# Tongji-MIC-Lab/TDVC

Hardware: AMD Instinct MI355X
Metric: 1080p P-frames/sec (encode + reconstruct, lambda=2048 config) (higher is better)
Workload: dtype f16; 1 GPU; 1x 1920x1080 (padded 1088x1920) 7-frame synthetic GOP (seed 1234), batch 1, P-frames coded in GOP order; gop=7, batch=1, parallelism=gop-sharded x1, weights=closed-form filler (no checkpoint ships)

## Files before the change

### include/tdvc_hip.h

```cpp
#ifndef TDVC_HIP_H
#define TDVC_HIP_H

#include <stdint.h>

#ifdef __cplusplus
extern "C" {
#endif

#define TDVC_OK 0
#define TDVC_EINVAL (-1)
#define TDVC_ENOSUP (-2)

typedef struct {
  void* p;
  int32_t N, H, W, C;
  int64_t sn;
  int32_t sp;
  int32_t dtype;
} tdvc_fmap;

enum { TDVC_F16 = 0, TDVC_F32 = 1 };
enum { TDVC_ACT_NONE = 0, TDVC_ACT_RELU = 1, TDVC_ACT_LRELU = 2, TDVC_ACT_CLAMP01 = 3, TDVC_ACT_SIGMOID = 4 };
enum { TDVC_GDN_NONE = 0, TDVC_GDN_FWD = 1, TDVC_GDN_INV = 2 };
enum { TDVC_OUT_NHWC = 0,
       TDVC_OUT_SHUFFLE2 = 1,
       TDVC_OUT_NCHW_F32 = 2 };

#define TDVC_MAX_TAPS 49

typedef struct {
  tdvc_fmap x;
  tdvc_fmap y;
  const void* w;
  const float* bias;
  int32_t cout;
  int32_t ntaps;
  int8_t tap_dy[TDVC_MAX_TAPS], tap_dx[TDVC_MAX_TAPS];
  int32_t kh, kw, stride, pad;
  int32_t ck;
  int32_t square_input;
  int32_t gdn;
  tdvc_fmap aux;
  int32_t act; float slope;
  int32_t round_before_act;
  tdvc_fmap res;
  tdvc_fmap res2;
  int32_t out_mode;
  int32_t s2d;
  int32_t bcast_T;
  float bcast_slope;
  float* chan_sum;
  tdvc_fmap flow;
} tdvc_conv_desc;

int tdvc_abi_version(void);
const char* tdvc_last_error(void);
int tdvc_prepare_device(void);
const char* tdvc_last_conv_kernel(void);

int tdvc_set_predicate(const int* flag);
int tdvc_last_launch_predicated(void);
#define TDVC_MAX_PREDICATE_IMAGES 4
int tdvc_set_predicate_images(const int* flags, int n);
int tdvc_frame_changed(const tdvc_fmap* cur, tdvc_fmap* cache, int* flag, void* stream);
int tdvc_frames_changed(const tdvc_fmap* cur, tdvc_fmap* cache, int* flags, unsigned force_mask, void* stream);


int tdvc_conv_plan(int cin, int kh, int kw, int stride);
int64_t tdvc_conv_packed_bytes(int cout, int cin, int ntaps, int ck);
int tdvc_pack_conv_weights(const float* w_oihw, int cout, int cin_real, int cin, int kh, int kw,
                           int ntaps, const int8_t* tap_dy, const int8_t* tap_dx, int ck, uint16_t* dst);
int tdvc_conv2d(const tdvc_conv_desc* d, void* stream);
int tdvc_conv_chan_sum_rows(const tdvc_conv_desc* d);
int tdvc_conv_flow_supported(const tdvc_conv_desc* d);
const char* tdvc_conv_select(const tdvc_conv_desc* d);
int tdvc_conv2d_f32(const tdvc_conv_desc* d, void* stream);

typedef struct {
  tdvc_fmap x, y;
  const void* w;
  const float* bias;
  int32_t act1; float slope1;
  int32_t act2; float slope2;
  int32_t add_input;
  tdvc_fmap res2;
} tdvc_conv_pair_desc;
int64_t tdvc_conv_pair_packed_bytes(void);
int tdvc_pack_conv_pair_weights(const float* w1_oihw, const float* w2_oihw, uint16_t* dst);
int tdvc_conv_pair_supported(const tdvc_conv_pair_desc* d);
int tdvc_conv_pair(const tdvc_conv_pair_desc* d, void* stream);

typedef struct {
  tdvc_fmap x, om, y;
  const void* w;
  const float* bias;
  int32_t groups;
  int32_t act; float slope; int32_t round_before_act;
  void* x_planar;
} tdvc_dcn_desc;
int tdvc_dcn_fused(const tdvc_dcn_desc* d, void* stream);

int tdvc_dcn_v2_forward_f32(const float* input, const float* weight, const float* bias,
                            const float* offset, const float* mask, float* output,
                            int B, int C, int H, int W, int Cout,
                            int kh, int kw, int sh, int sw, int ph, int pw, int dh, int dw,
                            int deformable_group, void* stream);
int tdvc_dcn_v2_backward_f32(const float* input, const float* weight, const float* bias,
                             const float* offset, const float* mask, const float* grad_output,
                             float* grad_input, float* grad_offset, float* grad_mask,
                             float* grad_weight, float* grad_bias, float* columns,
                             int B, int C, int H, int W, int Cout,
                             int kh, int kw, int sh, int sw, int ph, int pw, int dh, int dw,
                             int deformable_group, void* stream);

int tdvc_nchw_to_fmap(const float* src, int C, const tdvc_fmap* y, void* stream);
int tdvc_fmap_to_nchw(const tdvc_fmap* x, int C, float* dst, void* stream);
int tdvc_scale_act_res(const tdvc_fmap* a, const float* gate, int act, float slope,
                       const tdvc_fmap* r, float r_sign, const tdvc_fmap* y, const tdvc_fmap* y2, void* stream);
int tdvc_scale_act_res3(const tdvc_fmap* a, const float* gate, int act, float slope, const tdvc_fmap* r, float r_sign,
                        const tdvc_fmap* y, const tdvc_fmap* b, float b_sign, const tdvc_fmap* y3, void* stream);
int tdvc_add_flow(const tdvc_fmap* off, const tdvc_fmap* flow, void* stream);
int tdvc_bcast_add_act(const tdvc_fmap* x, const tdvc_fmap* b, int T, float slope, void* stream);

int tdvc_channel_sum(const tdvc_fmap* x, float* partial, int nblocks, void* stream);
int tdvc_se_gate(const float* partial, int nblocks, float inv_count, int N, int C, int Cmid,
                 const float* w1, const float* b1, const float* w2, const float* b2,
                 float* gate, void* stream);

int tdvc_upsample2x(const tdvc_fmap* x, const tdvc_fmap* y, void* stream);
int tdvc_avgpool2(const tdvc_fmap* x, const tdvc_fmap* y, void* stream);
int tdvc_avgpool2_pyramid(const tdvc_fmap* xa, const tdvc_fmap* xb, const tdvc_fmap* ya, const tdvc_fmap* yb, void* stream);
int tdvc_spynet_level_input(const tdvc_fmap* ref, const tdvc_fmap* supp, const tdvc_fmap* flow_lo,
                            const tdvc_fmap* flow_up, const tdvc_fmap* cat8, void* stream);
int tdvc_resize_bilinear(const tdvc_fmap* x, const tdvc_fmap* y, const float* chscale, void* stream);

int64_t tdvc_avgpool_k_work_floats(int N, int hp, int wp, int C, int scale);
int tdvc_avgpool_k(const tdvc_fmap* x, int scale, float* pooled, int hp, int wp, float* work, int64_t work_floats, void* stream);
int tdvc_patch_match(const float* pin, const float* pref, int N, int hp, int wp, int C,
                     int32_t* idx, void* stream);
int tdvc_match_gather(const tdvc_fmap* fin, const tdvc_fmap* fref, const int32_t* idx, int scale,
                      int hp, int wp, const tdvc_fmap* cat, void* stream);
// ... 176 lines not shown
```

### tdvc_amd/_lib.py

```python
from __future__ import annotations

import ctypes as C
import os

_HERE = os.path.dirname(os.path.abspath(__file__))
LIB_PATH = os.path.join(_HERE, "libtdvc_hip.so")

MAX_TAPS = 49
F16, F32 = 0, 1
ACT_NONE, ACT_RELU, ACT_LRELU, ACT_CLAMP01, ACT_SIGMOID = 0, 1, 2, 3, 4
GDN_NONE, GDN_FWD, GDN_INV = 0, 1, 2
OUT_NHWC, OUT_SHUFFLE2, OUT_NCHW_F32 = 0, 1, 2


class FMapDesc(C.Structure):
    _fields_ = [("p", C.c_void_p), ("N", C.c_int32), ("H", C.c_int32), ("W", C.c_int32), ("C", C.c_int32),
                ("sn", C.c_int64), ("sp", C.c_int32), ("dtype", C.c_int32)]


class ConvDesc(C.Structure):
    _fields_ = [("x", FMapDesc), ("y", FMapDesc), ("w", C.c_void_p), ("bias", C.c_void_p),
                ("cout", C.c_int32), ("ntaps", C.c_int32),
                ("tap_dy", C.c_int8 * MAX_TAPS), ("tap_dx", C.c_int8 * MAX_TAPS),
                ("kh", C.c_int32), ("kw", C.c_int32), ("stride", C.c_int32), ("pad", C.c_int32),
                ("ck", C.c_int32), ("square_input", C.c_int32), ("gdn", C.c_int32),
                ("aux", FMapDesc), ("act", C.c_int32), ("slope", C.c_float),
                ("round_before_act", C.c_int32), ("res", FMapDesc), ("res2", FMapDesc), ("out_mode", C.c_int32), ("s2d", C.c_int32),
                ("bcast_T", C.c_int32), ("bcast_slope", C.c_float), ("chan_sum", C.c_void_p), ("flow", FMapDesc)]


class DcnDesc(C.Structure):
    _fields_ = [("x", FMapDesc), ("om", FMapDesc), ("y", FMapDesc), ("w", C.c_void_p), ("bias", C.c_void_p),
                ("groups", C.c_int32), ("act", C.c_int32), ("slope", C.c_float), ("round_before_act", C.c_int32), ("x_planar", C.c_void_p)]


class ConvPairDesc(C.Structure):
    _fields_ = [("x", FMapDesc), ("y", FMapDesc), ("w", C.c_void_p), ("bias", C.c_void_p), ("act1", C.c_int32), ("slope1", C.c_float),
                ("act2", C.c_int32), ("slope2", C.c_float), ("add_input", C.c_int32), ("res2", FMapDesc)]


class WgradReduceJob(C.Structure):
    _fields_ = [("work", C.c_void_p), ("bwork", C.c_void_p), ("row_off", C.c_void_p), ("chan_off", C.c_void_p), ("tap_off", C.c_void_p),
                ("bias_index", C.c_void_p), ("dw", C.c_void_p), ("db", C.c_void_p), ("scale", C.c_float),
                ("nworkers", C.c_int32), ("cow", C.c_int32), ("ciw", C.c_int32), ("ntaps", C.c_int32), ("cout", C.c_int32), ("cin", C.c_int32),
                ("wblocks", C.c_int32), ("nblocks", C.c_int32)]


_P = C.c_void_p
_FM = C.POINTER(FMapDesc)
_i, _f, _i64 = C.c_int, C.c_float, C.c_int64

SIGNATURES = {
    "tdvc_abi_version": (_i, []),
    "tdvc_conv_chan_sum_rows": (_i, [C.POINTER(ConvDesc)]),
    "tdvc_conv_select": (C.c_char_p, [C.POINTER(ConvDesc)]),
    "tdvc_conv_flow_supported": (_i, [C.POINTER(ConvDesc)]),
    "tdvc_scale_act_res3": (_i, [_FM, _P, _i, _f, _FM, _f, _FM, _FM, _f, _FM, _P]),
    "tdvc_avgpool2_pyramid": (_i, [_FM, _FM, _FM, _FM, _P]),
    "tdvc_last_error": (C.c_char_p, []),
    "tdvc_last_conv_kernel": (C.c_char_p, []),
    "tdvc_prepare_device": (_i, []),
    "tdvc_set_predicate": (_i, [_P]),
    "tdvc_set_predicate_images": (_i, [_P, _i]),
    "tdvc_last_launch_predicated": (_i, []),
    "tdvc_frame_changed": (_i, [_FM, _FM, _P, _P]),
    "tdvc_frames_changed": (_i, [_FM, _FM, _P, C.c_uint, _P]),
    "tdvc_conv_plan": (_i, [_i, _i, _i, _i]),
    "tdvc_conv_packed_bytes": (_i64, [_i, _i, _i, _i]),
    "tdvc_pack_conv_weights": (_i, [_P, _i, _i, _i, _i, _i, _i, _P, _P, _i, _P]),
    "tdvc_conv2d": (_i, [C.POINTER(ConvDesc), _P]),
    "tdvc_conv2d_f32": (_i, [C.POINTER(ConvDesc), _P]),
    "tdvc_pack_conv_weights_indexed": (_i, [_P] * 7 + [_i] * 4 + [_P, _P]),
    "tdvc_pack_conv_weights_indexed_f32": (_i, [_P] * 7 + [_i] * 4 + [_P, _P]),
    "tdvc_pack_job_blocks": (_i64, [_i, _i, _i, _i]),
    "tdvc_pack_conv_weights_batch": (_i, [_P, _P, _i, _i, _P]),
    "tdvc_act_backward": (_i, [_FM, _FM, _FM, _i, _f, _FM, _P]),
    "tdvc_pixel_unshuffle": (_i, [_FM, _FM, _P]),
    "tdvc_bias_grad_work_floats": (_i64, [_i, _i]),
    "tdvc_bias_grad": (_i, [_FM, _i, _P, _f, _P, _P, _i64, _P]),
    "tdvc_copy_cast": (_i, [_FM, _FM, _P]),
    "tdvc_clamp01_backward": (_i, [_FM, _FM, _P]),
    "tdvc_gate_backward_work_floats": (_i64, [_i, _i]),
    "tdvc_gate_backward": (_i, [_FM, _FM, _P, _FM, _P, _P, _i64, _P]),
    "tdvc_se_gate_backward": (_i, [_P, _i, _f, _i, _i, _i] + [_P] * 6 + [_f] + [_P] * 6),
    "tdvc_bcast_channel_add": (_i, [_FM, _P, _f, _P]),
    "tdvc_add_flow_backward": (_i, [_FM, _FM, _P]),
    "tdvc_bcast_add_act_backward": (_i, [_FM, _FM, _FM, _f, _P]),
    "tdvc_upsample2x_backward": (_i, [_FM, _FM, _P]),
    "tdvc_resize_bilinear_backward": (_i, [_FM, _FM, _P, _P]),
    "tdvc_spynet_level_input_backward": (_i, [_FM, _FM, _FM, _FM, _FM, _P]),
    "tdvc_sigmoid_f32": (_i, [_P, _P, _i64, _P]),
    "tdvc_sigmoid_backward_f32": (_i, [_P, _P, _i64, _P]),
    "tdvc_axpy_f32": (_i, [_P, _P, _f, _i64, _P]),
    "tdvc_match_gather_backward": (_i, [_FM, _FM, _P, _i, _i, _i, _FM, _FM, _FM, _P]),
    "tdvc_eb_backward": (_i, [_FM, _P, _FM, _f, _FM, _P, _P]),
    "tdvc_eb_pack": (_i, [_P, _P, _P, _i, _P]),
    "tdvc_eb_param_chain": (_i, [_P, _P, _P, _f, _i, _P]),
    "tdvc_eb_aux": (_i, [_P, _P, _f, _P, _P, _i, _P]),
    "tdvc_gc_backward": (_i, [_FM, _FM, _FM, _f, _FM, _FM, _P]),
    "tdvc_dcn_columns": (_i, [_FM, _FM, _i, _FM, _P]),
    "tdvc_ar_lanes_state_bytes": (_i64, [_i]),
    "tdvc_ar_gather_batch": (_i, [_FM, _FM, _P, _i, _FM, _FM, _P]),
    "tdvc_ar_quantize_batch": (_i, [_FM, _FM, _P, _i, _P, _i, _P, _FM, _P, _P, _i64, _P]),
    "tdvc_ar_indexes_batch": (_i, [_FM, _P, _i, _i, _P, _i, _i, _i, _i, _P, _i64, _P]),
    "tdvc_ar_wavefront_batch": (_i, [_P, _P, _i, _P, _i, _P, _P, _FM, _FM, _FM, _FM, _FM, _P, _i, _FM, _P, _P, _i, _i, _i, _P, _i, _P, _P, _P]),
    "tdvc_ar_decode_serial_batch": (_i, [_P, _P, _i, _P, _i, _P, _P, _FM, _FM, _FM, _FM, _P, _i, _FM, _P, _i, _i, _i, _P, _i, _P, _P, _P]),
    "tdvc_ar_lanes_batch_layout": (_i64, [_P, _i, _i, _P]),
    "tdvc_ar_lanes_init_batch": (_i, [_P, _i64, _P, _i, _i, _P, _P]),
    "tdvc_ar_decode_lanes_step_batch": (_i, [_FM, _P, _i, _P, _i, _P, _i64, _P, _i, _P, C.c_int32, _P, _P, _P, C.c_int32, _P, _FM, _P, _P, _i64, _P]),
    "tdvc_ar_wavefront_lanes_batch": (_i, [_P, _P, _i, _P, _i64, _P, _P, C.c_int32, _P, _P, _P, C.c_int32, _FM, _FM, _FM, _FM, _P, _i, _FM, _P, _P, _i, _i, _i,
                                           _P, _i, _P, _P, _P, _P]),
    "tdvc_ar_encode_lanes_scratch_words": (_i64, [_i64, _i, _i]),
    "tdvc_ar_encode_lanes_out_bytes": (_i64, [_i64, _i, _i]),
    "tdvc_ar_encode_lanes_batch": (_i, [_P, _P, _i, _i, _i, _i, _P, _i, _i, _P, C.c_int32, _P, _P, _P, C.c_int32, _P, _i64, _i64, _P, _i64, _i64, _P, _P]),
    "tdvc_rans_encode_lanes_dev_ref": (_i, [_P, _P, _i, _i, _i, _i, _P, _i, _i, _P, C.c_int32, _P, _P, C.c_int32, _P, _i64, _i64, _P, _i64, _i64, _P]),
    "tdvc_ar_last_loop_launches": (_i64, []),
    "tdvc_ssim_level_work_floats": (_i64, [_i] * 5),
    "tdvc_ssim_level": (_i, [_P, _P, _i, _i, _i, _i, _P, _i, _f, _f, _P, _P, _P, _i64, _P]),
    "tdvc_avgpool2_pad_f32": (_i, [_P, _i64, _i, _i, _P, _P]),
    "tdvc_ssim_level_backward": (_i, [_P, _P, _i, _i, _i, _i, _P, _i, _f, _f, _P, _P, _f, _P, _P, _P]),
    "tdvc_msssim_level_grads": (_i, [_P, _P, _P, _i, _i, _P, _P, _P, _P, _P]),
    "tdvc_dcn_col2im_work_floats": (_i64, [_i, _i, _i, _i]),
    "tdvc_dcn_col2im": (_i, [_FM, _FM, _FM, _i, _P, _FM, _P, _i64, _P]),
    "tdvc_dcn_col2im_det": (_i, [_FM, _FM, _FM, _i, _P, _FM, _P, _i64, _P, _P, _P, _i, _P]),
    "tdvc_dcn_far_apply": (_i, [_P, _P, _P, _i, _P, _P]),
    "tdvc_conv_wgrad_work_floats": (_i64, [_i] * 6),
    "tdvc_conv_wgrad": (_i, [_FM, _FM] + [_i] * 6 + [_P] * 5 + [_i, _f, _P, _P, _i64, _P]),
    "tdvc_conv_wgrad_bias": (_i, [_FM, _FM] + [_i] * 6 + [_P] * 5 + [_i, _f, _P, _P, _P, _P, _i64, _P]),
    "tdvc_conv_wgrad_partials": (_i, [_FM, _FM] + [_i] * 6 + [_P] * 5 + [_i, _f, _P, _P, _P, _P, _i64, C.POINTER(WgradReduceJob), _P]),
    "tdvc_wgrad_reduce_batch": (_i, [_P, _P, _i, _i, _P]),
    "tdvc_gdn_backward": (_i, [_FM, _FM, _FM, _i, _FM, _FM, _P]),
    "tdvc_mul2_accumulate": (_i, [_FM, _FM, _FM, _P]),
    "tdvc_dcn_fused": (_i, [C.POINTER(DcnDesc), _P]),
    "tdvc_conv_pair_packed_bytes": (_i64, []),
    "tdvc_pack_conv_pair_weights": (_i, [_P, _P, _P]),
    "tdvc_conv_pair_supported": (_i, [C.POINTER(ConvPairDesc)]),
    "tdvc_conv_pair": (_i, [C.POINTER(ConvPairDesc), _P]),
    "tdvc_dcn_v2_forward_f32": (_i, [_P] * 6 + [_i] * 14 + [_P]),
    "tdvc_dcn_v2_backward_f32": (_i, [_P] * 12 + [_i] * 14 + [_P]),
    "tdvc_nchw_to_fmap": (_i, [_P, _i, _FM, _P]),
    "tdvc_fmap_to_nchw": (_i, [_FM, _i, _P, _P]),
    "tdvc_scale_act_res": (_i, [_FM, _P, _i, _f, _FM, _f, _FM, _FM, _P]),
    "tdvc_add_flow": (_i, [_FM, _FM, _P]),
# ... 57 lines not shown
```

### tdvc_amd/csrc/conv_common.h

```cpp
#pragma once
#include "common.h"

namespace convk {

struct ConvParams {
  const half_t* x; long x_sn; int x_sp; int H, W, Cin;
  const half_t* w; const float* bias;
  FMap y; int Ho, Wo; int cout;
  FMap aux; FMap res; FMap res2;
  int ntaps, kh, kw, pad;
  int in_stride;
  int nchunks, steps;
  int square, gdn, act; float slope; int round16, out_mode;
  int tiles_x;
  int simple;
  int s2d, Corig;
  int reverse;
  int bcast_T; float bcast_slope;
  float* csum;
  int8_t tap_dy[TDVC_MAX_TAPS], tap_dx[TDVC_MAX_TAPS];
  const int* pred;
  FMap flow;
};

enum ConvSwitch { SW_NONE = -1, SW_V2, SW_V3, SW_V5, SW_V7, SW_V9, SW_V10, SW_V11, SW_ROW, SW_C8, SW_N16, SW_GDN128, SW_HEAD3, SW_COUNT };
int conv_on(int id);
long conv_v9_work_limit();

constexpr long LARGE_MAP_PIXELS = 8192;

inline bool taps_dense(const tdvc_conv_desc* d, int kh, int kw, int pad) {
  if (d->ntaps != kh * kw || d->kh != kh || d->kw != kw || d->pad != pad) return false;
  for (int t = 0; t < d->ntaps; ++t)
    if (d->tap_dy[t] != t / kw || d->tap_dx[t] != t % kw) return false;
  return true;
}

inline bool all_waves_store(const tdvc_conv_desc* d, int wave_ch) {
  const int ych = d->out_mode == TDVC_OUT_SHUFFLE2 ? d->cout >> 2 : (d->cout + wave_ch - 1) / wave_ch * wave_ch;
  return d->y.C > ych - wave_ch;
}

inline int persistent_grid_x(int slots, int cout_blocks, int N, int ntiles) {
  const int gx = slots / (cout_blocks * N);
  return gx < 1 ? 1 : (gx > ntiles ? ntiles : gx);
}

template <auto Kern, typename... Args>
int launch_big_lds(const char* what, int lds_limit, dim3 grid, dim3 block, int lds, hipStream_t st, Args... args) {
  static TdvcPerDeviceFlag raised;
  bool& done = raised.flag();
  if (!done) {
    const hipError_t err = hipFuncSetAttribute(reinterpret_cast<const void*>(Kern), hipFuncAttributeMaxDynamicSharedMemorySize, lds_limit);
    if (err != hipSuccess) { tdvc_set_error("%s: hipFuncSetAttribute failed: %s", what, hipGetErrorString(err)); return (int)err; }
    done = true;
  }
  hipLaunchKernelGGL(Kern, grid, block, lds, st, args...);
  return tdvc_launch_status(what);
}


template <bool F32MAPS = false>
__device__ __forceinline__ void epilogue4(const ConvParams& p, int n, int oy, int ox, int co, float v[4]) {
  if (p.bias) {
    const f32x4 b4 = *reinterpret_cast<const f32x4*>(p.bias + co);
#pragma unroll
    for (int i = 0; i < 4; ++i) v[i] += b4[i];
  }
  int py = oy, px = ox, pc = co, PW = p.Wo;
  if (p.out_mode == TDVC_OUT_SHUFFLE2) {
    const int cq = p.cout >> 2;
    const int sub = co / cq;
    pc = co - sub * cq;
    py = 2 * oy + (sub >> 1);
    px = 2 * ox + (sub & 1);
    PW = 2 * p.Wo;
  }
  if (p.gdn) {
    float a[4];
    if (F32MAPS && p.aux.f32) {
      const f32x4 a4 = *reinterpret_cast<const f32x4*>(reinterpret_cast<const float*>(p.aux.p) + (long)n * p.aux.sn + ((long)oy * p.Wo + ox) * p.aux.sp + co);
#pragma unroll
      for (int i = 0; i < 4; ++i) v[i] = a4[i] * (p.gdn == TDVC_GDN_FWD ? 1.0f / sqrtf(v[i]) : sqrtf(v[i]));
    } else {
      const half4 a4 = *reinterpret_cast<const half4*>(reinterpret_cast<const half_t*>(p.aux.p) + (long)n * p.aux.sn + ((long)oy * p.Wo + ox) * p.aux.sp + co);
#pragma unroll
      for (int i = 0; i < 4; ++i) a[i] = (float)a4[i];
#pragma unroll
      for (int i = 0; i < 4; ++i) v[i] = a[i] * (p.gdn == TDVC_GDN_FWD ? rsqrtf(v[i]) : sqrtf(v[i]));
    }
  }
  if (p.round16) {
#pragma unroll
    for (int i = 0; i < 4; ++i) v[i] = (float)(half_t)v[i];
  }
  if (p.act) {
#pragma unroll
    for (int i = 0; i < 4; ++i) v[i] = act_apply(v[i], p.act, p.slope);
  }
  const long opix = (long)py * PW + px;
  if (p.res.p) {
    if (p.res.f32) {
      const float* rp = reinterpret_cast<const float*>(p.res.p) + (long)n * p.res.sn + opix * p.res.sp + pc;
#pragma unroll
      for (int i = 0; i < 4; ++i)
        if (pc + i < p.res.C) v[i] += rp[i];
    } else if (pc < p.res.C) {
      const half4 r4 = *reinterpret_cast<const half4*>(reinterpret_cast<const half_t*>(p.res.p) + (long)n * p.res.sn + opix * p.res.sp + pc);
// ... 326 lines not shown
```

### tdvc_amd/csrc/conv_dispatch.hip

```cpp
#include <stdlib.h>

#include "conv_common.h"

using convk::ConvParams;
bool conv_v2_eligible(const tdvc_conv_desc* d, int Ho, int Wo); int launch_conv_v2(const ConvParams& p, int cout_blocks, int N, hipStream_t st);
bool conv_v3_eligible(const tdvc_conv_desc* d, int Ho, int Wo); int launch_conv_v3(const ConvParams& p, int cout_blocks, int N, hipStream_t st);
bool conv_v5_eligible(const tdvc_conv_desc* d, int Ho, int Wo); int launch_conv_v5(const ConvParams& p, int cout_blocks, int N, hipStream_t st); int conv_v5_chan_sum_rows(int Ho, int Wo, int cout_blocks, int N);
bool conv_v7_eligible(const tdvc_conv_desc* d, const ConvParams& p, int Ho, int Wo); int launch_conv_v7(const ConvParams& p, int cout_blocks, int N, hipStream_t st);
bool conv_v9_eligible(const tdvc_conv_desc* d, int Ho, int Wo, bool v3_ok); int launch_conv_v9(const ConvParams& p, int ck8, int cout_tiles32, int N, hipStream_t st);
bool conv_v10_eligible(const tdvc_conv_desc* d, const ConvParams& p, int Ho, int Wo); int launch_conv_v10(const ConvParams& p, int cout_blocks, int N, hipStream_t st);
bool conv_v11_eligible(const tdvc_conv_desc* d, const ConvParams& p, int Ho, int Wo); int launch_conv_v11(const ConvParams& p, int cout_blocks, int N, hipStream_t st);
int conv_row_geometry(const tdvc_conv_desc* d, const ConvParams& p, int Ho, int Wo); int launch_conv_row(int geo, const ConvParams& p, int N, hipStream_t st);
bool conv_c8_eligible(const tdvc_conv_desc* d, const ConvParams& p, int Ho, int Wo); int launch_conv_c8(const ConvParams& p, int N, hipStream_t st);
bool conv_n16_eligible(const tdvc_conv_desc* d, int Ho, int Wo); int launch_conv_n16(const ConvParams& p, int N, hipStream_t st);
bool gdn128_eligible(const tdvc_conv_desc* d, const ConvParams& p, int Ho, int Wo); int launch_gdn128(const ConvParams& p, int N, hipStream_t st);
int conv_direct_lds_bytes(const tdvc_conv_desc* d);
int conv_cout_tiles(int cout);
int launch_conv_direct(const ConvParams& p, int ck8, int stride, int N, hipStream_t st);
int conv_f32_validate(const tdvc_conv_desc* d, int& Ho, int& Wo);

namespace {
const char* const kSwitchEnv[convk::SW_COUNT] = {nullptr, "TDVC_CONV_NO_V3", "TDVC_CONV_NO_V5", "TDVC_CONV_NO_V7", "TDVC_CONV_NO_V9", "TDVC_CONV_NO_V10",
                                                 "TDVC_CONV_NO_V11", "TDVC_CONV_NO_ROW", "TDVC_CONV_NO_C8", "TDVC_CONV_NO_N16", "TDVC_CONV_NO_GDN128", "TDVC_CONV_NO_HEAD3"};
int g_enabled[convk::SW_COUNT] = {1, 1, 1, 1, 1, 1, 1, 15, 1, 1, 1, 1};
long g_v9_work_limit = 1L << 20;
}

int convk::conv_on(int id) {
  static const struct EnvOff {
    bool off[convk::SW_COUNT];
    EnvOff() {
      const bool v1 = getenv("TDVC_CONV_V1") != nullptr;
      for (int i = 0; i < convk::SW_COUNT; ++i) off[i] = v1 || (kSwitchEnv[i] && getenv(kSwitchEnv[i]) != nullptr);
    }
  } env;
  return id == convk::SW_NONE ? 1 : (env.off[id] ? 0 : g_enabled[id]);
}
long convk::conv_v9_work_limit() { return g_v9_work_limit; }

extern "C" void tdvc_debug_enable_conv_v9(int enable) { g_enabled[convk::SW_V9] = enable != 0; }
extern "C" void tdvc_debug_enable_conv_v10(int enable) { g_enabled[convk::SW_V10] = enable != 0; }
extern "C" void tdvc_debug_enable_conv_v11(int enable) { g_enabled[convk::SW_V11] = enable != 0; }
extern "C" void tdvc_debug_enable_conv_row(int mask) { g_enabled[convk::SW_ROW] = mask; }
extern "C" void tdvc_debug_enable_conv_c8(int enable) { g_enabled[convk::SW_C8] = enable != 0; }
extern "C" void tdvc_debug_enable_conv_n16(int enable) { g_enabled[convk::SW_N16] = enable != 0; }
extern "C" void tdvc_debug_enable_gdn128(int enable) { g_enabled[convk::SW_GDN128] = enable != 0; }
extern "C" void tdvc_debug_enable_conv_head3(int enable) { g_enabled[convk::SW_HEAD3] = enable != 0; }
extern "C" void tdvc_debug_set_conv_v9_work_limit(long v) { g_v9_work_limit = v; }

namespace {

struct Pick {
  const tdvc_conv_desc* d;
  int Ho, Wo;
  int geo;
  int ck8() const { return d->ck / 8; }
  int N() const { return d->x.N; }
  int cout_blocks() const { return conv_cout_tiles(d->cout) / 2; }
};

struct Entry {
  const char* name;
  int sw;
  bool (*eligible)(Pick& k, const ConvParams& p);
  int (*launch)(const Pick& k, const ConvParams& p, hipStream_t st);
  bool (*only)(const tdvc_conv_desc* d);
  const char* only_msg;
};

bool v3_on_and_eligible(const Pick& k) { return convk::conv_on(convk::SW_V3) && conv_v3_eligible(k.d, k.Ho, k.Wo); }

bool bcast_eligible(Pick& k, const ConvParams& p) {
  const tdvc_conv_desc* d = k.d;
  return d->bcast_T == 4 && d->kh == 1 && d->kw == 1 && d->stride == 1 && d->pad == 0 && d->cout == 64 && d->y.C == 64 && d->y.sp >= 4 * 64 &&
         d->y.dtype == TDVC_F16 && d->out_mode == TDVC_OUT_NHWC && d->act == TDVC_ACT_NONE && !d->gdn && !d->res2.p &&
         (!d->res.p || (d->res.dtype == TDVC_F16 && d->res.C == 64 && d->res.sp >= 4 * 64 && d->res.N == d->y.N && d->res.H == d->y.H && d->res.W == d->y.W)) &&
         !d->square_input && !d->round_before_act && d->bias && d->bcast_slope >= 0.f && d->bcast_slope <= 1.f && conv_v5_eligible(d, k.Ho, k.Wo) &&
         convk::conv_is_lean(p);
}
int bcast_launch(const Pick& k, const ConvParams& p, hipStream_t st) {
  ConvParams q = p;
  q.simple = 2;
  q.slope = 1.f;
  return launch_conv_v5(q, 1, k.N(), st);
}
bool row_eligible(Pick& k, const ConvParams& p) { return (k.geo = conv_row_geometry(k.d, p, k.Ho, k.Wo)) >= 0; }

constexpr char kNameV5[] = "conv_mfma_v5", kNameDirect[] = "conv_mfma<%d,%d,%d>";

const Entry kTable[] = {
    {"conv_mfma_v5(bcast)", convk::SW_V5, bcast_eligible, bcast_launch, [](const tdvc_conv_desc* d) { return d->bcast_T != 0; },
     "tdvc_conv2d: bcast_T needs a plain 1x1 / stride 1 conv to 64 channels of >= 8192 pixels, y (and res, the optional source of the slices) a 64-channel window of a buffer with >= 4 slices, bcast_T == 4"},
    {"conv_row(s2d)", convk::SW_ROW, [](Pick& k, const ConvParams& p) { return k.d->s2d && row_eligible(k, p); },
     [](const Pick& k, const ConvParams& p, hipStream_t st) { return launch_conv_row(k.geo, p, k.N(), st); }, nullptr, nullptr},
    {"conv_mfma_v3(s2d)", convk::SW_V3, [](Pick& k, const ConvParams&) { return k.d->s2d && conv_v3_eligible(k.d, k.Ho, k.Wo); },
     [](const Pick& k, const ConvParams& p, hipStream_t st) { return launch_conv_v3(p, k.cout_blocks(), k.N(), st); },
     [](const tdvc_conv_desc* d) { return d->s2d != 0; }, "tdvc_conv2d: s2d conv not eligible for the stage-pipelined kernel"},
    {"conv_mfma_v9", convk::SW_V9, [](Pick& k, const ConvParams&) { return conv_v9_eligible(k.d, k.Ho, k.Wo, v3_on_and_eligible(k)); },
     [](const Pick& k, const ConvParams& p, hipStream_t st) { return launch_conv_v9(p, k.ck8(), conv_cout_tiles(k.d->cout), k.N(), st); }, nullptr, nullptr},
    {"gdn128", convk::SW_GDN128, [](Pick& k, const ConvParams& p) { return gdn128_eligible(k.d, p, k.Ho, k.Wo); },
     [](const Pick& k, const ConvParams& p, hipStream_t st) { return launch_gdn128(p, k.N(), st); }, nullptr, nullptr},
    {kNameV5, convk::SW_V5, [](Pick& k, const ConvParams&) { return conv_v5_eligible(k.d, k.Ho, k.Wo); },
     [](const Pick& k, const ConvParams& p, hipStream_t st) { return launch_conv_v5(p, k.cout_blocks(), k.N(), st); }, nullptr, nullptr},
    {"conv_c8", convk::SW_C8, [](Pick& k, const ConvParams& p) { return conv_c8_eligible(k.d, p, k.Ho, k.Wo); },
     [](const Pick& k, const ConvParams& p, hipStream_t st) { return launch_conv_c8(p, k.N(), st); }, nullptr, nullptr},
    {"conv_n16", convk::SW_N16, [](Pick& k, const ConvParams&) { return conv_n16_eligible(k.d, k.Ho, k.Wo); },
     [](const Pick& k, const ConvParams& p, hipStream_t st) { return launch_conv_n16(p, k.N(), st); }, nullptr, nullptr},
    {"conv_row", convk::SW_ROW, row_eligible,
     [](const Pick& k, const ConvParams& p, hipStream_t st) { return launch_conv_row(k.geo, p, k.N(), st); }, nullptr, nullptr},
    {"conv_mfma_v10", convk::SW_V10, [](Pick& k, const ConvParams& p) { return conv_v10_eligible(k.d, p, k.Ho, k.Wo); },
     [](const Pick& k, const ConvParams& p, hipStream_t st) { return launch_conv_v10(p, k.cout_blocks(), k.N(), st); }, nullptr, nullptr},
    {"conv_mfma_v7", convk::SW_V7, [](Pick& k, const ConvParams& p) { return conv_v7_eligible(k.d, p, k.Ho, k.Wo); },
     [](const Pick& k, const ConvParams& p, hipStream_t st) { return launch_conv_v7(p, k.cout_blocks(), k.N(), st); }, nullptr, nullptr},
    {"conv_mfma_v11", convk::SW_V11, [](Pick& k, const ConvParams& p) { return conv_v11_eligible(k.d, p, k.Ho, k.Wo); },
     [](const Pick& k, const ConvParams& p, hipStream_t st) { return launch_conv_v11(p, k.cout_blocks(), k.N(), st); }, nullptr, nullptr},
    {"conv_mfma_v3", convk::SW_V3, [](Pick& k, const ConvParams&) { return conv_v3_eligible(k.d, k.Ho, k.Wo); },
     [](const Pick& k, const ConvParams& p, hipStream_t st) { return launch_conv_v3(p, k.cout_blocks(), k.N(), st); }, nullptr, nullptr},
    {"conv_mfma_v2", convk::SW_V2, [](Pick& k, const ConvParams&) { return conv_v2_eligible(k.d, k.Ho, k.Wo); },
     [](const Pick& k, const ConvParams& p, hipStream_t st) { return launch_conv_v2(p, k.cout_blocks(), k.N(), st); }, nullptr, nullptr},
    {kNameDirect, convk::SW_NONE, [](Pick& k, const ConvParams&) { return conv_direct_lds_bytes(k.d) <= 64 * 1024; },
     [](const Pick& k, const ConvParams& p, hipStream_t st) { return launch_conv_direct(p, k.ck8(), k.d->stride, k.N(), st); },
     [](const tdvc_conv_desc*) { return true; }, nullptr},
};

const Entry* select(Pick& k, const ConvParams& p) {
  for (const Entry& e : kTable) {
    if (convk::conv_on(e.sw) && e.eligible(k, p)) return &e;
    if (e.only && e.only(k.d)) {
      if (e.only_msg) tdvc_set_error("%s", e.only_msg);
      else tdvc_set_error("tdvc_conv2d: LDS plan %d bytes too large for the direct kernel (use tdvc_conv_plan)", conv_direct_lds_bytes(k.d));
// ... 162 lines not shown
```

### tdvc_amd/csrc/conv_n16.hip

```cpp
#include "conv_common.h"

using convk::ConvParams;

namespace {

constexpr int N16_TH = 8, N16_TW = 64, N16_NTHR = 512;

struct N16Extra {
  int ksteps;
  int ps;
  int a_bytes;
  int ntiles, tiles_x;
  int cin_shift;
};

template <int NCB>
__global__ __launch_bounds__(N16_NTHR, 1) void conv_n16_kernel(const ConvParams p, const N16Extra e) {
  extern __shared__ __attribute__((aligned(16))) unsigned char smem[];
  unsigned char* wl = smem;
  unsigned char* tile = wl + e.a_bytes;
  const int tid = threadIdx.x, lane = tid & 63;
  const int wave = __builtin_amdgcn_readfirstlane(tid >> 6);
  const int px = lane & 15, kg = lane >> 4;
  const int TIW = N16_TW + p.kw - 1, TIH = N16_TH + p.kh - 1;
// ... 16 lines not shown
    return base + (dy * TIW + dx) * e.ps + (kk0 & (cin - 1)) * 2;
  };

  for (int tile_i = blockIdx.x; tile_i < e.ntiles; tile_i += gridDim.x) {
    const int per_img = e.tiles_x * ((p.Ho + N16_TH - 1) / N16_TH);
    const int n = tile_i / per_img, rem = tile_i - n * per_img;
    const int ty = rem / e.tiles_x, tx = rem - ty * e.tiles_x;
    const half_t* xn = p.x + (long)n * p.x_sn;
    const int iy0 = ty * N16_TH - p.pad, ix0 = tx * N16_TW - p.pad;
    __syncthreads();
    const int total = TIH * TIW * c8n;
    for (int idx0 = tid; idx0 < total; idx0 += 8 * N16_NTHR) {
      half8 v[8];
#pragma unroll
      for (int u = 0; u < 8; ++u) {
        const int idx = idx0 + u * N16_NTHR;
        const int pix = idx >> (e.cin_shift - 3), c8 = idx & (c8n - 1);
        const int rr = pix / TIW, cc = pix - rr * TIW;
        const int iy = iy0 + rr, ix = ix0 + cc;
        const bool ok = (int)(idx < total) & (int)(iy >= 0) & (int)(iy < p.H) & (int)(ix >= 0) & (int)(ix < p.W);
        const half_t* src = xn + ((long)(ok ? iy : 0) * p.W + (ok ? ix : 0)) * p.x_sp + c8 * 8;
        typedef unsigned u32x4 __attribute__((ext_vector_type(4)));
        u32x4 bits = *reinterpret_cast<const u32x4*>(src);
        unsigned m = ok ? 0xFFFFFFFFu : 0u;
        asm volatile("" : "+v"(m));
        bits &= m;
        v[u] = __builtin_bit_cast(half8, bits);
      }
#pragma unroll
      for (int u = 0; u < 8; ++u) {
        const int idx = idx0 + u * N16_NTHR;
        if (idx < total) {
          const int pix = idx >> (e.cin_shift - 3), c8 = idx & (c8n - 1);
          *reinterpret_cast<half8*>(tile + pix * e.ps + c8 * 16) = v[u];
        }
      }
    }
    __syncthreads();

    f32x4 acc[NCB][4];
#pragma unroll
    for (int cb = 0; cb < NCB; ++cb)
#pragma unroll
      for (int c = 0; c < 4; ++c) acc[cb][c] = f32x4{0.f, 0.f, 0.f, 0.f};

    half8 a0[NCB], b0[4], a1[NCB], b1[4];
    auto load = [&](int S, half8 (&a)[NCB], half8 (&b)[4]) {
      const int off = frag_off(S);
#pragma unroll
      for (int cb = 0; cb < NCB; ++cb) a[cb] = *reinterpret_cast<const half8*>(wl + ((S * NCB + cb) * 64 + lane) * 16);
#pragma unroll
      for (int c = 0; c < 4; ++c) b[c] = *reinterpret_cast<const half8*>(tile + off + c * cstep);
    };
    auto mm = [&](half8 (&a)[NCB], half8 (&b)[4]) {
#pragma unroll
      for (int c = 0; c < 4; ++c)
#pragma unroll
        for (int cb = 0; cb < NCB; ++cb) acc[cb][c] = __builtin_amdgcn_mfma_f32_16x16x32_f16(a[cb], b[c], acc[cb][c], 0, 0, 0);
    };
    const int KS = e.ksteps;
    load(0, a0, b0);
    for (int S = 0; S < KS; S += 2) {
      load(min(S + 1, KS - 1), a1, b1);
      mm(a0, b0);
      load(min(S + 2, KS - 1), a0, b0);
      if (S + 1 < KS) mm(a1, b1);
    }

    const int oy = ty * N16_TH + wave;
#pragma unroll
    for (int c = 0; c < 4; ++c) {
      const int ox = tx * N16_TW + 16 * c + px;
      if (oy < p.Ho && ox < p.Wo) {
#pragma unroll
        for (int cb = 0; cb < NCB; ++cb) {
          float v[4] = {acc[cb][c][0], acc[cb][c][1], acc[cb][c][2], acc[cb][c][3]};
          convk::epilogue4(p, n, oy, ox, 16 * cb + 4 * kg, v);
        }
      }
    }
  }
}

inline int n16_ps(int cin) { return 2 * cin + 16; }
inline int n16_ksteps(int ntaps, int cin) { return (ntaps * cin + 31) / 32; }
inline int n16_lds(int cin, int kh, int kw, int ntaps, int ncb) {
  return n16_ksteps(ntaps, cin) * ncb * 1024 + (N16_TH + kh - 1) * (N16_TW + kw - 1) * n16_ps(cin);
}

}

bool conv_n16_eligible(const tdvc_conv_desc* d, int Ho, int Wo) {
  const int cin = d->x.C;
  const bool cin_ok = cin == 8 || cin == 16 || cin == 32 || cin == 64;
  const bool dense = convk::taps_dense(d, d->kh, d->kw, d->pad);
  return cin_ok && dense && d->ck == cin && d->stride == 1 && d->cout <= 32 && !d->s2d && !d->square_input && !d->gdn &&
         (long)Ho * Wo >= convk::LARGE_MAP_PIXELS &&
         n16_lds(cin, d->kh, d->kw, d->ntaps, d->cout <= 16 ? 1 : 2) <= 150 * 1024;
}

bool conv_head3_takes(const ConvParams& p);
int launch_conv_head3(const ConvParams& p, int N, hipStream_t st);
static thread_local int g_n16_last_form = 0;
extern "C" int tdvc_debug_conv_n16_last_form(void) { return g_n16_last_form; }

int launch_conv_n16(const ConvParams& p, int N, hipStream_t st) {
  g_n16_last_form = convk::conv_on(convk::SW_HEAD3) && conv_head3_takes(p);
  if (g_n16_last_form) return launch_conv_head3(p, N, st);
  const int ncb = p.cout <= 16 ? 1 : 2;
  N16Extra e;
  e.ksteps = n16_ksteps(p.ntaps, p.Cin);
  e.ps = n16_ps(p.Cin);
  e.a_bytes = e.ksteps * ncb * 1024;
  e.tiles_x = (p.Wo + N16_TW - 1) / N16_TW;
  e.ntiles = N * e.tiles_x * ((p.Ho + N16_TH - 1) / N16_TH);
  e.cin_shift = p.Cin == 8 ? 3 : p.Cin == 16 ? 4 : p.Cin == 32 ? 5 : 6;
  const int lds = n16_lds(p.Cin, p.kh, p.kw, p.ntaps, ncb);
  const int per_cu = lds <= 78 * 1024 ? 2 : 1;
  int grid = e.ntiles < 256 * per_cu ? e.ntiles : 256 * per_cu;
  const auto go = ncb == 1 ? convk::launch_big_lds<&conv_n16_kernel<1>, ConvParams, N16Extra> : convk::launch_big_lds<&conv_n16_kernel<2>, ConvParams, N16Extra>;
  return go("tdvc_conv2d(n16)", 160 * 1024, dim3(grid), dim3(N16_NTHR), lds, st, p, e);
}
```

Measured before the change: 52.15 frames/s.

## Add register-prefetched streaming variant of n16 conv kernel overlapping next tile loads

Adds a persistent n16 conv kernel that loads the next tile's input into registers while the MFMA loop for the current tile runs, then writes it to LDS after a barrier. Bias is preloaded into registers and added before the epilogue. The goal is to hide global-load latency between tiles in the persistent loop. The cost is more register pressure from PT prefetch vectors under launch_bounds(…,1), plus an extra barrier per tile. The kernel is enabled by default, and a debug knob to force per-CU occupancy is added.

```diff
diff --git a/include/tdvc_hip.h b/include/tdvc_hip.h
--- a/include/tdvc_hip.h
+++ b/include/tdvc_hip.h
@@ -57,6 +57,8 @@
 const char* tdvc_last_error(void);
 int tdvc_prepare_device(void);
 const char* tdvc_last_conv_kernel(void);
+void tdvc_debug_enable_conv_n16_stream(int enable);
+int tdvc_debug_conv_n16_last_stream(void);
 
 int tdvc_set_predicate(const int* flag);
 int tdvc_last_launch_predicated(void);
diff --git a/tdvc_amd/_lib.py b/tdvc_amd/_lib.py
--- a/tdvc_amd/_lib.py
+++ b/tdvc_amd/_lib.py
@@ -59,6 +59,8 @@
     "tdvc_avgpool2_pyramid": (_i, [_FM, _FM, _FM, _FM, _P]),
     "tdvc_last_error": (C.c_char_p, []),
     "tdvc_last_conv_kernel": (C.c_char_p, []),
+    "tdvc_debug_enable_conv_n16_stream": (None, [_i]),
+    "tdvc_debug_conv_n16_last_stream": (_i, []),
     "tdvc_prepare_device": (_i, []),
     "tdvc_set_predicate": (_i, [_P]),
     "tdvc_set_predicate_images": (_i, [_P, _i]),
diff --git a/tdvc_amd/csrc/conv_common.h b/tdvc_amd/csrc/conv_common.h
--- a/tdvc_amd/csrc/conv_common.h
+++ b/tdvc_amd/csrc/conv_common.h
@@ -23,7 +23,7 @@
   FMap flow;
 };
 
-enum ConvSwitch { SW_NONE = -1, SW_V2, SW_V3, SW_V5, SW_V7, SW_V9, SW_V10, SW_V11, SW_ROW, SW_C8, SW_N16, SW_GDN128, SW_HEAD3, SW_COUNT };
+enum ConvSwitch { SW_NONE = -1, SW_V2, SW_V3, SW_V5, SW_V7, SW_V9, SW_V10, SW_V11, SW_ROW, SW_C8, SW_N16, SW_GDN128, SW_HEAD3, SW_N16_STREAM, SW_COUNT };
 int conv_on(int id);
 long conv_v9_work_limit();
 
diff --git a/tdvc_amd/csrc/conv_dispatch.hip b/tdvc_amd/csrc/conv_dispatch.hip
--- a/tdvc_amd/csrc/conv_dispatch.hip
+++ b/tdvc_amd/csrc/conv_dispatch.hip
@@ -21,8 +21,9 @@
 
 namespace {
 const char* const kSwitchEnv[convk::SW_COUNT] = {nullptr, "TDVC_CONV_NO_V3", "TDVC_CONV_NO_V5", "TDVC_CONV_NO_V7", "TDVC_CONV_NO_V9", "TDVC_CONV_NO_V10",
-                                                 "TDVC_CONV_NO_V11", "TDVC_CONV_NO_ROW", "TDVC_CONV_NO_C8", "TDVC_CONV_NO_N16", "TDVC_CONV_NO_GDN128", "TDVC_CONV_NO_HEAD3"};
-int g_enabled[convk::SW_COUNT] = {1, 1, 1, 1, 1, 1, 1, 15, 1, 1, 1, 1};
+                                                 "TDVC_CONV_NO_V11", "TDVC_CONV_NO_ROW", "TDVC_CONV_NO_C8", "TDVC_CONV_NO_N16", "TDVC_CONV_NO_GDN128", "TDVC_CONV_NO_HEAD3",
+                                                 "TDVC_CONV_NO_N16_STREAM"};
+int g_enabled[convk::SW_COUNT] = {1, 1, 1, 1, 1, 1, 1, 15, 1, 1, 1, 1, 1};
 long g_v9_work_limit = 1L << 20;
 }
 
@@ -46,6 +47,7 @@
 extern "C" void tdvc_debug_enable_conv_n16(int enable) { g_enabled[convk::SW_N16] = enable != 0; }
 extern "C" void tdvc_debug_enable_gdn128(int enable) { g_enabled[convk::SW_GDN128] = enable != 0; }
 extern "C" void tdvc_debug_enable_conv_head3(int enable) { g_enabled[convk::SW_HEAD3] = enable != 0; }
+extern "C" void tdvc_debug_enable_conv_n16_stream(int enable) { g_enabled[convk::SW_N16_STREAM] = enable != 0; }
 extern "C" void tdvc_debug_set_conv_v9_work_limit(long v) { g_v9_work_limit = v; }
 
 namespace {
diff --git a/tdvc_amd/csrc/conv_n16.hip b/tdvc_amd/csrc/conv_n16.hip
--- a/tdvc_amd/csrc/conv_n16.hip
+++ b/tdvc_amd/csrc/conv_n16.hip
@@ -122,6 +122,140 @@
   }
 }
 
+template <int NCB, int PT>
+__global__ __launch_bounds__(N16_NTHR, 1) void conv_n16_stream_kernel(const ConvParams p, const N16Extra e) {
+  typedef unsigned u32x4 __attribute__((ext_vector_type(4)));
+  extern __shared__ __attribute__((aligned(16))) unsigned char smem[];
+  unsigned char* wl = smem;
+  unsigned char* tile = wl + e.a_bytes;
+  const int tid = threadIdx.x, lane = tid & 63;
+  const int wave = __builtin_amdgcn_readfirstlane(tid >> 6);
+  const int px = lane & 15, kg = lane >> 4;
+  const int TIW = N16_TW + p.kw - 1, TIH = N16_TH + p.kh - 1;
+  const int cin = p.Cin, c8n = cin >> 3;
+  const int total = TIH * TIW * c8n;
+  const int per_img = e.tiles_x * ((p.Ho + N16_TH - 1) / N16_TH);
+
+  u32x4 treg[PT];
+  unsigned okmask = 0u;
+  auto issue = [&](int tile_i) {
+    const int n = tile_i / per_img, rem = tile_i - n * per_img;
+    const int ty = rem / e.tiles_x, tx = rem - ty * e.tiles_x;
+    const half_t* xn = p.x + (long)n * p.x_sn;
+    const int iy0 = ty * N16_TH - p.pad, ix0 = tx * N16_TW - p.pad;
+    unsigned m = 0u;
+#pragma unroll
+    for (int u = 0; u < PT; ++u) {
+      const int idx = tid + u * N16_NTHR;
+      const int pix = idx >> (e.cin_shift - 3), c8 = idx & (c8n - 1);
+      const int rr = pix / TIW, cc = pix - rr * TIW;
+      const int iy = iy0 + rr, ix = ix0 + cc;
+      const bool ok = (int)(idx < total) & (int)(iy >= 0) & (int)(iy < p.H) & (int)(ix >= 0) & (int)(ix < p.W);
+      const half_t* src = xn + ((long)(ok ? iy : 0) * p.W + (ok ? ix : 0)) * p.x_sp + c8 * 8;
+      treg[u] = *reinterpret_cast<const u32x4*>(src);
+      m |= (ok ? 1u : 0u) << u;
+    }
+    okmask = m;
+  };
+  auto publish = [&]() {
+#pragma unroll
+    for (int u = 0; u < PT; ++u) {
+      const int idx = tid + u * N16_NTHR;
+      const int pix = idx >> (e.cin_shift - 3), c8 = idx & (c8n - 1);
+      const u32x4 z = {0u, 0u, 0u, 0u};
+      const u32x4 val = ((okmask >> u) & 1u) ? treg[u] : z;
+      if (idx < total) *reinterpret_cast<u32x4*>(tile + pix * e.ps + c8 * 16) = val;
+    }
+  };
+
+  const int base = (wave * TIW + px) * e.ps;
+  const int cstep = 16 * e.ps;
+  auto frag_off = [&](int S) {
+    const int kk0 = 32 * S + 8 * kg;
+    const int tap = min(kk0 >> e.cin_shift, p.ntaps - 1);
+    const int dy = tap / p.kw, dx = tap - dy * p.kw;
+    return base + (dy * TIW + dx) * e.ps + (kk0 & (cin - 1)) * 2;
+  };
+
+  f32x4 b4[NCB];
+#pragma unroll
+  for (int cb = 0; cb < NCB; ++cb) b4[cb] = p.bias ? *reinterpret_cast<const f32x4*>(p.bias + 16 * cb + 4 * kg) : f32x4{0.f, 0.f, 0.f, 0.f};
+  ConvParams pe = p;
+  pe.bias = nullptr;
+
+  for (int i = tid; i < e.ksteps * NCB * 64; i += N16_NTHR) {
+    const int ln = i & 63, cb = (i >> 6) % NCB, S = (i >> 6) / NCB;
+    const int q = 4 * S + (ln >> 4), s = q >> 1, h = q & 1;
+    half8 v = {0, 0, 0, 0, 0, 0, 0, 0};
+    if (s < p.steps) v = *reinterpret_cast<const half8*>(p.w + ((long)s * 64 + (16 * cb + (ln & 15)) + 32 * h) * 8);
+    *reinterpret_cast<half8*>(wl + (long)i * 16) = v;
+  }
+
+  int tile_i = blockIdx.x;
+  if (tile_i < e.ntiles) issue(tile_i);
+  auto arrived = [&]() {
+#pragma unroll
+    for (int u = 0; u < PT; ++u) asm volatile("" : "+v"(treg[u]));
+  };
+  arrived();
+  for (; tile_i < e.ntiles; tile_i += gridDim.x) {
+    const int n = tile_i / per_img, rem = tile_i - n * per_img;
+    const int ty = rem / e.tiles_x, tx = rem - ty * e.tiles_x;
+    publish();
+    __syncthreads();
+    if (tile_i + (int)gridDim.x < e.ntiles) issue(tile_i + gridDim.x);
+
+    f32x4 acc[NCB][4];
+#pragma unroll
+    for (int cb = 0; cb < NCB; ++cb)
+#pragma unroll
+      for (int c = 0; c < 4; ++c) acc[cb][c] = f32x4{0.f, 0.f, 0.f, 0.f};
+
+    half8 a0[NCB], b0[4], a1[NCB], b1[4];
+    auto load = [&](int S, half8 (&a)[NCB], half8 (&b)[4]) {
+      const int off = frag_off(S);
+#pragma unroll
+      for (int cb = 0; cb < NCB; ++cb) a[cb] = *reinterpret_cast<const half8*>(wl + ((S * NCB + cb) * 64 + lane) * 16);
+#pragma unroll
+      for (int c = 0; c < 4; ++c) b[c] = *reinterpret_cast<const half8*>(tile + off + c * cstep);
+    };
+    auto mm = [&](half8 (&a)[NCB], half8 (&b)[4]) {
+#pragma unroll
+      for (int c = 0; c < 4; ++c)
+#pragma unroll
+        for (int cb = 0; cb < NCB; ++cb) acc[cb][c] = __builtin_amdgcn_mfma_f32_16x16x32_f16(a[cb], b[c], acc[cb][c], 0, 0, 0);
+    };
+    const int KS = e.ksteps;
+    load(0, a0, b0);
+    for (int S = 0; S < KS; S += 2) {
+      load(min(S + 1, KS - 1), a1, b1);
+      mm(a0, b0);
+      load(min(S + 2, KS - 1), a0, b0);
+      if (S + 1 < KS) mm(a1, b1);
+    }
+
+    arrived();
+
+    const int oy = ty * N16_TH + wave;
+#pragma unroll
+    for (int c = 0; c < 4; ++c) {
+      const int ox = tx * N16_TW + 16 * c + px;
+      if (oy < p.Ho && ox < p.Wo) {
+#pragma unroll
+        for (int cb = 0; cb < NCB; ++cb) {
+          float v[4] = {acc[cb][c][0], acc[cb][c][1], acc[cb][c][2], acc[cb][c][3]};
+          if (p.bias) {
+#pragma unroll
+            for (int i = 0; i < 4; ++i) v[i] += b4[cb][i];
+          }
+          convk::epilogue4(pe, n, oy, ox, 16 * cb + 4 * kg, v);
+        }
+      }
+    }
+    __syncthreads();
+  }
+}
+
 inline int n16_ps(int cin) { return 2 * cin + 16; }
 inline int n16_ksteps(int ntaps, int cin) { return (ntaps * cin + 31) / 32; }
 inline int n16_lds(int cin, int kh, int kw, int ntaps, int ncb) {
@@ -144,10 +278,32 @@
 static thread_local int g_n16_last_form = 0;
 extern "C" int tdvc_debug_conv_n16_last_form(void) { return g_n16_last_form; }
 
+static thread_local int g_n16_last_stream = 0;
+extern "C" int tdvc_debug_conv_n16_last_stream(void) { return g_n16_last_stream; }
+static int g_n16_per_cu = 0;
+extern "C" void tdvc_debug_set_conv_n16_per_cu(int per_cu) { g_n16_per_cu = per_cu; }
+
+namespace {
+using N16Launch = int (*)(const char*, int, dim3, dim3, int, hipStream_t, ConvParams, N16Extra);
+template <int NCB>
+N16Launch n16_stream_launcher(int pt) {
+  switch (pt) {
+    case 2: return convk::launch_big_lds<&conv_n16_stream_kernel<NCB, 2>, ConvParams, N16Extra>;
+    case 4: return convk::launch_big_lds<&conv_n16_stream_kernel<NCB, 4>, ConvParams, N16Extra>;
+    case 8: return convk::launch_big_lds<&conv_n16_stream_kernel<NCB, 8>, ConvParams, N16Extra>;
+    default: return convk::launch_big_lds<&conv_n16_stream_kernel<NCB, 11>, ConvParams, N16Extra>;
+  }
+}
+}
+
 int launch_conv_n16(const ConvParams& p, int N, hipStream_t st) {
   g_n16_last_form = convk::conv_on(convk::SW_HEAD3) && conv_head3_takes(p);
+  g_n16_last_stream = 0;
   if (g_n16_last_form) return launch_conv_head3(p, N, st);
   const int ncb = p.cout <= 16 ? 1 : 2;
+  const int pieces = ((N16_TH + p.kh - 1) * (N16_TW + p.kw - 1) * (p.Cin / 8) + N16_NTHR - 1) / N16_NTHR;
+  const int pt = pieces <= 2 ? 2 : pieces <= 4 ? 4 : pieces <= 8 ? 8 : pieces <= 11 ? 11 : 0;
+  g_n16_last_stream = pt != 0 && convk::conv_on(convk::SW_N16_STREAM);
   N16Extra e;
   e.ksteps = n16_ksteps(p.ntaps, p.Cin);
   e.ps = n16_ps(p.Cin);
@@ -156,8 +312,10 @@
   e.ntiles = N * e.tiles_x * ((p.Ho + N16_TH - 1) / N16_TH);
   e.cin_shift = p.Cin == 8 ? 3 : p.Cin == 16 ? 4 : p.Cin == 32 ? 5 : 6;
   const int lds = n16_lds(p.Cin, p.kh, p.kw, p.ntaps, ncb);
-  const int per_cu = lds <= 78 * 1024 ? 2 : 1;
+  int per_cu = lds <= 78 * 1024 ? 2 : 1;
+  if (g_n16_per_cu == 1 || (g_n16_per_cu == 2 && lds <= 78 * 1024)) per_cu = g_n16_per_cu;
   int grid = e.ntiles < 256 * per_cu ? e.ntiles : 256 * per_cu;
-  const auto go = ncb == 1 ? convk::launch_big_lds<&conv_n16_kernel<1>, ConvParams, N16Extra> : convk::launch_big_lds<&conv_n16_kernel<2>, ConvParams, N16Extra>;
+  N16Launch go = ncb == 1 ? convk::launch_big_lds<&conv_n16_kernel<1>, ConvParams, N16Extra> : convk::launch_big_lds<&conv_n16_kernel<2>, ConvParams, N16Extra>;
+  if (g_n16_last_stream) go = ncb == 1 ? n16_stream_launcher<1>(pt) : n16_stream_launcher<2>(pt);
   return go("tdvc_conv2d(n16)", 160 * 1024, dim3(grid), dim3(N16_NTHR), lds, st, p, e);
 }
```

New measurement: 52.36 frames/s (median of 6 runs). No clear change (+0.4%).
